# harskish/ganspace

Hardware: NVIDIA H100
Metric: latent samples/sec into PCA (StyleGAN2-ffhq W, N=1e6) (higher is better)
Workload: dtype f32

## Files before the change

### ganspace_b200/csrc/subspace.cu

```cuda
#include "ipca_internal.cuh"
#include <math.h>
#include <stdlib.h>
#include <string.h>

namespace gsb {

constexpr int SC_CL = 16;
constexpr int SC_WARPS = 8;
constexpr int SC_THREADS = SC_WARPS * 32;
constexpr int SC_KT = 32;
constexpr int SC_LDA = SC_KT + 4;
constexpr int SC_STAGES = 3;
constexpr int SC_NB = 5;
constexpr int SC_MAXG = 2;

struct SubspaceParams {
    double *hdr, *mean, *unnorm, *H, *Qbuf;
    const double *mean_b, *gram_b;
    double *Gt, *Part, *Red, *Slots;
    double *Prof;
    int d, c;
    double n_seen, n_b, tol;
    double dbl;
    int maxit;
    int *status;
};

__device__ __forceinline__ void dmma884(double &c0, double &c1, double a, double b) {
    asm("mma.sync.aligned.m8n8k4.row.col.f64.f64.f64.f64 {%0,%1}, {%2}, {%3}, {%0,%1};" : "+d"(c0), "+d"(c1) : "d"(a), "d"(b));
}
__device__ __forceinline__ void sc_cluster_sync() {
    asm volatile("barrier.cluster.arrive.release.aligned;" ::: "memory");
    asm volatile("barrier.cluster.wait.acquire.aligned;" ::: "memory");
}
__device__ __forceinline__ void cp_async16(double *dst, const double *src) {
    const unsigned sa = (unsigned)__cvta_generic_to_shared(dst);
    asm volatile("cp.async.cg.shared.global [%0], [%1], 16;" ::"r"(sa), "l"(src) : "memory");
}
__device__ __forceinline__ void cta_copy_async(double *dst, const double *src, int ndoubles) {
    for (int ch = threadIdx.x; ch < ndoubles / 2; ch += SC_THREADS) cp_async16(dst + 2 * ch, src + 2 * ch);
}

template <bool AT, bool BT>
__device__ __forceinline__ void mma_group(const double *__restrict__ As, int lda, const double *__restrict__ Bs, int ldb,
                                          int ksteps, int m0, int n0, int nb, double (&acc)[SC_NB][2]) {
    const int lane = threadIdx.x & 31, g = lane >> 2, t = lane & 3;
    const double *ap = AT ? (As + (size_t)t * lda + m0 + g) : (As + (size_t)(m0 + g) * lda + t);
    const double *bp = BT ? (Bs + (size_t)(n0 + g) * ldb + t) : (Bs + (size_t)t * ldb + n0 + g);
    const int astep = AT ? 4 * lda : 4, bstep = BT ? 4 : 4 * ldb, bnext = BT ? 8 * ldb : 8;
#pragma unroll 2
    for (int ks = 0; ks < ksteps; ++ks) {
        const double a = ap[(size_t)ks * astep];
#pragma unroll
        for (int b = 0; b < SC_NB; ++b) {
            if (b < nb) {
                const double bv = bp[(size_t)ks * bstep + (size_t)b * bnext];
                dmma884(acc[b][0], acc[b][1], a, bv);
            }
        }
    }
}

__device__ __forceinline__ double fast_rsqrt(double x) {
    double y;
    asm("rsqrt.approx.ftz.f64 %0, %1;" : "=d"(y) : "d"(x));
    const double h = 0.5 * x;
    double t = fma(-h * y, y, 0.5);
    y = fma(y, t, y);
    t = fma(-h * y, y, 0.5);
    y = fma(y, t, y);
    return y;
}

__device__ __forceinline__ void zero_acc(double (&acc)[SC_NB][2]) {
#pragma unroll
    for (int b = 0; b < SC_NB; ++b) { acc[b][0] = 0.0; acc[b][1] = 0.0; }
}

struct Grouping { int mt, nt, nbsel, ngroups; };
__device__ __forceinline__ Grouping make_grouping(int mt, int nt) {
    Grouping q;
    q.mt = mt; q.nt = nt;
    int nb = (mt * nt + SC_WARPS - 1) / SC_WARPS;
    nb = nb < 1 ? 1 : (nb > SC_NB ? SC_NB : nb);
    q.nbsel = nb;
    q.ngroups = mt * ((nt + nb - 1) / nb);
    return q;
}


template <int RA, int CB>
__device__ __forceinline__ void chol_solve_blocked(const double *__restrict__ Ws, double *__restrict__ Ys, int c, int cp, int RPC,
                                                   double *__restrict__ buf ) {
    const int tid = threadIdx.x, ry = tid >> 4, cx = tid & 15, lane = tid & 31;
    const int nrows = c + RPC, CL = 16 * RA;
    double *P = buf, *XS = buf + (size_t)CL * 9, *Lb = XS + (size_t)CL * 9;
    double A[RA][CB];
#pragma unroll
    for (int a = 0; a < RA; ++a) {
        const int r = ry + 16 * a;
#pragma unroll
        for (int b = 0; b < CB; ++b) {
            const int q = cx + 16 * b;
            double v = 0.0;
            if (r < nrows && q < c) v = (r < c) ? Ws[(size_t)r * cp + q] : Ys[(size_t)(r - c) * cp + q];
            A[a][b] = v;
        }
    }
    const double floor_ = fmax(fabs(Ws[0]) * 1e-26, 1e-300);
    __syncthreads();
    for (int p = 0; p < c / 8; ++p) {
        const int j0 = 8 * p, pb = p >> 1, pc = (p & 1) * 8;
        if (cx >= pc && cx < pc + 8) {
#pragma unroll
            for (int b = 0; b < CB; ++b)
                if (b == pb) {
#pragma unroll
                    for (int a = 0; a < RA; ++a) P[(size_t)(ry + 16 * a) * 9 + (cx - pc)] = A[a][b];
                }
        }
        __syncthreads();
        if (tid < 32) {
            const int l = lane & 7;
            double row[8];
#pragma unroll
            for (int k = 0; k < 8; ++k) row[k] = P[(size_t)(j0 + l) * 9 + k];
#pragma unroll
            for (int j = 0; j < 8; ++j) {
                double piv = __shfl_sync(0xffffffffu, row[j], j);
                if (!(piv > floor_)) piv = floor_;
                const double inv = fast_rsqrt(piv);
                const double lij = row[j] * inv;
#pragma unroll
                for (int k = j + 1; k < 8; ++k) {
                    const double lkj = __shfl_sync(0xffffffffu, lij, k);
                    row[k] = fma(-lij, lkj, row[k]);
                }
                row[j] = lij;
                if (lane == j) Lb[72 + j] = inv;
            }
            if (lane < 8) {
#pragma unroll
                for (int k = 0; k < 8; ++k) Lb[l * 9 + k] = (k <= l) ? row[k] : 0.0;
            }
        }
        __syncthreads();
        for (int r = j0 + 8 + tid; r < nrows; r += SC_THREADS) {
            double x[8];
#pragma unroll
            for (int k = 0; k < 8; ++k) {
                double sacc = P[(size_t)r * 9 + k];
#pragma unroll
                for (int m = 0; m < k; ++m) sacc = fma(-x[m], Lb[k * 9 + m], sacc);
                x[k] = sacc * Lb[72 + k];
            }
#pragma unroll
            for (int k = 0; k < 8; ++k) XS[(size_t)r * 9 + k] = x[k];
            if (r >= c) {
#pragma unroll
                for (int k = 0; k < 8; ++k) Ys[(size_t)(r - c) * cp + j0 + k] = x[k];
            }
        }
        __syncthreads();
        double xr[RA][8];
#pragma unroll
        for (int a = 0; a < RA; ++a) {
            const int r = ry + 16 * a;
            const bool ok = (r >= j0 + 8) && (r < nrows);
#pragma unroll
            for (int k = 0; k < 8; ++k) xr[a][k] = ok ? XS[(size_t)r * 9 + k] : 0.0;
        }
#pragma unroll
        for (int b = 0; b < CB; ++b) {
            const int q = cx + 16 * b;
            if (q >= j0 + 8 && q < c) {
                double xq[8];
#pragma unroll
                for (int k = 0; k < 8; ++k) xq[k] = XS[(size_t)q * 9 + k];
#pragma unroll
                for (int a = 0; a < RA; ++a) {
                    double v = A[a][b];
#pragma unroll
                    for (int k = 0; k < 8; ++k) v = fma(-xr[a][k], xq[k], v);
                    A[a][b] = v;
                }
            }
        }
    }
    __syncthreads();
}

template <int RA, int CB>
__global__ void __launch_bounds__(SC_THREADS, 1)
subspace_step_kernel(const SubspaceParams p) {
    extern __shared__ __align__(16) double sc_smem[];
    const int d = p.d, c = p.c, cp = c + 4, RPC = d / SC_CL, RT = RPC / 8, CT = c / 8, nkt = d / SC_KT;
    const int tid = threadIdx.x, lane = tid & 31, warp = tid >> 5, fg = lane >> 2, ft = lane & 3;
    uint32_t me_u;
    asm volatile("mov.u32 %0, %%cluster_ctarank;" : "=r"(me_u));
    const int me = (int)me_u;

    double *As = sc_smem;
    double *Bs = As + (size_t)SC_STAGES * RPC * SC_LDA;
    double *Ys = Bs + (size_t)SC_STAGES * SC_KT * cp;
    double *Qq = Ys + (size_t)RPC * cp;
    double *Ws = Qq + (size_t)RPC * cp;
    double *mv = Ws + (size_t)c * cp;
    double *red = mv + d;
    double *cholbuf = red + 64;
    long long tprev = clock64();
    double prof[10] = {0, 0, 0, 0, 0, 0, 0, 0, 0, 0};
#define PROF(k) do { const long long tn_ = clock64(); prof[k] += (double)(tn_ - tprev); tprev = tn_; } while (0)

    const double n_seen = p.n_seen, n_b = p.n_b, n_tot = n_seen + n_b;
    int cur = (int)__ldcg(p.hdr + 3);
    double *Qc = p.Qbuf + (size_t)cur * d * cp, *Qn = p.Qbuf + (size_t)(cur ^ 1) * d * cp;
    const size_t tileA = (size_t)RPC * SC_LDA, tileB = (size_t)SC_KT * cp;
    double *Gmine = p.Gt + (size_t)me * nkt * tileA;

    {
        const double f = sqrt((n_seen / n_tot) * n_b);
        for (int i = tid; i < d; i += SC_THREADS) mv[i] = f * (__ldcg(p.mean + i) - __ldcg(p.mean_b + i));
        const double *src = Qc + (size_t)me * RPC * cp;
        for (int i = tid; i < RPC * cp; i += SC_THREADS) Qq[i] = __ldcg(src + i);
        for (int i = tid; i < c * c; i += SC_THREADS) Ws[(i / c) * cp + i % c] = __ldcg(p.H + i);
    }
    __syncthreads();
    {
        const Grouping gr = make_grouping(RT, CT);
        for (int g = warp; g < gr.ngroups; g += SC_WARPS) {
            const int rt = g % gr.mt, ct0 = (g / gr.mt) * gr.nbsel;
            const int nb = (gr.nt - ct0 < gr.nbsel) ? gr.nt - ct0 : gr.nbsel;
            double acc[SC_NB][2];
            zero_acc(acc);
            mma_group<false, false>(Qq, cp, Ws, cp, c / 4, rt * 8, ct0 * 8, nb, acc);
#pragma unroll
            for (int b = 0; b < SC_NB; ++b)
                if (b < nb) {
                    double *o = Ys + (size_t)(rt * 8 + fg) * cp + (ct0 + b) * 8 + 2 * ft;
                    o[0] = acc[b][0]; o[1] = acc[b][1];
                }
        }
    }
    __syncthreads();
    PROF(0);
    {
        const Grouping gr = make_grouping(RT, SC_KT / 8);
        auto copy_c = [&](int stage, int kt_) {
            double *dstc = As + (size_t)stage * tileA;
            for (int ch = tid; ch < RPC * (SC_KT / 2); ch += SC_THREADS) {
                const int r = ch / (SC_KT / 2), o2 = ch % (SC_KT / 2);
                cp_async16(dstc + (size_t)r * SC_LDA + 2 * o2, p.gram_b + (size_t)(me * RPC + r) * d + kt_ * SC_KT + 2 * o2);
            }
        };
        for (int s = 0; s < SC_STAGES - 1; ++s) {
            if (s < nkt) { cta_copy_async(Bs + (size_t)s * tileB, Qc + (size_t)s * tileB, (int)tileB); copy_c(s, s); }
            asm volatile("cp.async.commit_group;" ::: "memory");
        }
        for (int kt = 0; kt < nkt; ++kt) {
            asm volatile("cp.async.wait_group %0;" ::"n"(SC_STAGES - 2) : "memory");
            __syncthreads();
            {
                const int nx = kt + SC_STAGES - 1;
                if (nx < nkt) {
                    cta_copy_async(Bs + (size_t)(nx % SC_STAGES) * tileB, Qc + (size_t)nx * tileB, (int)tileB);
                    copy_c(nx % SC_STAGES, nx);
                }
                asm volatile("cp.async.commit_group;" ::: "memory");
            }
            const double *Bt = Bs + (size_t)(kt % SC_STAGES) * tileB, *Cst = As + (size_t)(kt % SC_STAGES) * tileA;
            for (int g = warp; g < gr.ngroups; g += SC_WARPS) {
                const int rt = g % gr.mt, ct0 = (g / gr.mt) * gr.nbsel;
                const int nb = (gr.nt - ct0 < gr.nbsel) ? gr.nt - ct0 : gr.nbsel;
                double acc[SC_NB][2];
                zero_acc(acc);
                mma_group<false, true>(Ys, cp, Bt, cp, c / 4, rt * 8, ct0 * 8, nb, acc);
                const int lrow = rt * 8 + fg, grow = me * RPC + lrow;
                const double mr = mv[grow];
#pragma unroll
                for (int b = 0; b < SC_NB; ++b)
                    if (b < nb) {
                        const int lcol = (ct0 + b) * 8 + 2 * ft, gcol = kt * SC_KT + lcol;
                        const double2 cb = *reinterpret_cast<const double2 *>(Cst + (size_t)lrow * SC_LDA + lcol);
                        double2 o;
                        o.x = acc[b][0] + cb.x + mr * mv[gcol];
                        o.y = acc[b][1] + cb.y + mr * mv[gcol + 1];
                        *reinterpret_cast<double2 *>(Gmine + (size_t)kt * tileA + (size_t)lrow * SC_LDA + lcol) = o;
                    }
            }
        }
        asm volatile("cp.async.wait_group 0;" ::: "memory");
    }
    __syncthreads();
    PROF(1);

    const Grouping gy = make_grouping(RT, CT);
    const Grouping gh = make_grouping(CT, CT);
    const int E = 2 * c * c, slice = (E + SC_CL - 1) / SC_CL;
    double rel = 0.0;
    int it = 0;
    bool conv = false;
    auto gemm_into_ys = [&](const double *Bsrc) {
        {
        double acc[SC_MAXG][SC_NB][2];
#pragma unroll
        for (int q = 0; q < SC_MAXG; ++q) zero_acc(acc[q]);
        for (int s = 0; s < SC_STAGES - 1; ++s) {
            if (s < nkt) {
                cta_copy_async(As + (size_t)s * tileA, Gmine + (size_t)s * tileA, (int)tileA);
                cta_copy_async(Bs + (size_t)s * tileB, Bsrc + (size_t)s * tileB, (int)tileB);
            }
            asm volatile("cp.async.commit_group;" ::: "memory");
        }
        for (int kt = 0; kt < nkt; ++kt) {
            asm volatile("cp.async.wait_group %0;" ::"n"(SC_STAGES - 2) : "memory");
            __syncthreads();
            {
                const int nx = kt + SC_STAGES - 1;
                if (nx < nkt) {
                    cta_copy_async(As + (size_t)(nx % SC_STAGES) * tileA, Gmine + (size_t)nx * tileA, (int)tileA);
                    cta_copy_async(Bs + (size_t)(nx % SC_STAGES) * tileB, Bsrc + (size_t)nx * tileB, (int)tileB);
                }
                asm volatile("cp.async.commit_group;" ::: "memory");
            }
            const double *At = As + (size_t)(kt % SC_STAGES) * tileA, *Bt = Bs + (size_t)(kt % SC_STAGES) * tileB;
#pragma unroll
            for (int q = 0; q < SC_MAXG; ++q) {
                const int g = warp + q * SC_WARPS;
                if (g < gy.ngroups) {
                    const int rt = g % gy.mt, ct0 = (g / gy.mt) * gy.nbsel;
                    const int nb = (gy.nt - ct0 < gy.nbsel) ? gy.nt - ct0 : gy.nbsel;
                    mma_group<false, false>(At, SC_LDA, Bt, cp, SC_KT / 4, rt * 8, ct0 * 8, nb, acc[q]);
                }
            }
        }
        asm volatile("cp.async.wait_group 0;" ::: "memory");
#pragma unroll
        for (int q = 0; q < SC_MAXG; ++q) {
            const int g = warp + q * SC_WARPS;
            if (g < gy.ngroups) {
                const int rt = g % gy.mt, ct0 = (g / gy.mt) * gy.nbsel;
                const int nb = (gy.nt - ct0 < gy.nbsel) ? gy.nt - ct0 : gy.nbsel;
#pragma unroll
                for (int b = 0; b < SC_NB; ++b)
                    if (b < nb) {
                        double *o = Ys + (size_t)(rt * 8 + fg) * cp + (ct0 + b) * 8 + 2 * ft;
                        o[0] = acc[q][b][0]; o[1] = acc[q][b][1];
                    }
            }
        }
    }
    };
    auto partial_reduce = [&]() {
    {
        double *Ph = p.Part + (size_t)me * E, *Pw = Ph + (size_t)c * c;
        for (int g = warp; g < gh.ngroups; g += SC_WARPS) {
            const int mt = g % gh.mt, ct0 = (g / gh.mt) * gh.nbsel;
            const int nb = (gh.nt - ct0 < gh.nbsel) ? gh.nt - ct0 : gh.nbsel;
            double ah[SC_NB][2], aw[SC_NB][2];
            zero_acc(ah); zero_acc(aw);
            mma_group<true, false>(Qq, cp, Ys, cp, RPC / 4, mt * 8, ct0 * 8, nb, ah);
            mma_group<true, false>(Ys, cp, Ys, cp, RPC / 4, mt * 8, ct0 * 8, nb, aw);
#pragma unroll
            for (int b = 0; b < SC_NB; ++b)
                if (b < nb) {
                    const size_t o = (size_t)(mt * 8 + fg) * c + (ct0 + b) * 8 + 2 * ft;
                    *reinterpret_cast<double2 *>(Ph + o) = make_double2(ah[b][0], ah[b][1]);
                    *reinterpret_cast<double2 *>(Pw + o) = make_double2(aw[b][0], aw[b][1]);
                }
        }
    }
    __syncthreads();
    sc_cluster_sync();
    for (int q0 = 0; q0 < slice; q0 += 4 * SC_THREADS) {
        double v[4][SC_CL];
#pragma unroll
        for (int u = 0; u < 4; ++u) {
            const int el = me * slice + q0 + u * SC_THREADS + tid;
            const bool ok = (q0 + u * SC_THREADS + tid < slice) && el < E;
#pragma unroll
            for (int r = 0; r < SC_CL; ++r) v[u][r] = ok ? __ldcg(p.Part + (size_t)r * E + el) : 0.0;
        }
#pragma unroll
        for (int u = 0; u < 4; ++u) {
            const int el = me * slice + q0 + u * SC_THREADS + tid;
            if ((q0 + u * SC_THREADS + tid < slice) && el < E) {
                double s = 0.0;
#pragma unroll
                for (int r = 0; r < SC_CL; ++r) s += v[u][r];
                p.Red[el] = s;
            }
        }
    }
    __syncthreads();
    sc_cluster_sync();
    };
    for (;;) {
        gemm_into_ys(Qc);
        __syncthreads();
        PROF(2);
        partial_reduce();
        for (int i = tid; i < c * c; i += SC_THREADS) Ws[(i / c) * cp + i % c] = __ldcg(p.Red + i);
        __syncthreads();
        PROF(4);
        double rs = 0.0;
        for (int g = warp; g < gy.ngroups; g += SC_WARPS) {
            const int rt = g % gy.mt, ct0 = (g / gy.mt) * gy.nbsel;
            const int nb = (gy.nt - ct0 < gy.nbsel) ? gy.nt - ct0 : gy.nbsel;
            double acc[SC_NB][2];
            zero_acc(acc);
            mma_group<false, false>(Qq, cp, Ws, cp, c / 4, rt * 8, ct0 * 8, nb, acc);
#pragma unroll
            for (int b = 0; b < SC_NB; ++b)
                if (b < nb) {
                    const double *y = Ys + (size_t)(rt * 8 + fg) * cp + (ct0 + b) * 8 + 2 * ft;
                    const double r0 = y[0] - acc[b][0], r1 = y[1] - acc[b][1];
                    rs = fma(r0, r0, rs);
                    rs = fma(r1, r1, rs);
                }
        }
        rs = block_sum(rs, red);
        if (tid == 0) p.Slots[me] = rs;
        __syncthreads();
        sc_cluster_sync();
        {
            double sl[SC_CL];
#pragma unroll
            for (int r = 0; r < SC_CL; ++r) sl[r] = __ldcg(p.Slots + r);
            double hmin = 1e300;
            for (int i = lane; i < c; i += 32) hmin = fmin(hmin, Ws[(size_t)i * cp + i]);
            for (int o = 16; o > 0; o >>= 1) hmin = fmin(hmin, __shfl_xor_sync(0xffffffffu, hmin, o));
            double tot = 0.0;
#pragma unroll
            for (int r = 0; r < SC_CL; ++r) tot += sl[r];
            rel = (hmin > 0.0) ? sqrt(tot) / hmin : 1e300;
            conv = rel <= p.tol;
        }
        PROF(5);
        if (conv || it >= p.maxit) break;
        ++it;
        if (rel > p.dbl * p.tol && it < p.maxit) {
            double *dst = Qn + (size_t)me * RPC * cp;
            for (int i = tid; i < RPC * cp; i += SC_THREADS) dst[i] = ((i % cp) < c) ? Ys[i] : 0.0;
            __syncthreads();
            sc_cluster_sync();
            gemm_into_ys(Qn);
            __syncthreads();
            partial_reduce();
            ++it;
            PROF(2);
        }
        for (int i = tid; i < c * c; i += SC_THREADS) Ws[(i / c) * cp + i % c] = __ldcg(p.Red + (size_t)c * c + i);
        __syncthreads();
        chol_solve_blocked<RA, CB>(Ws, Ys, c, cp, RPC, cholbuf);
        PROF(6);
        {
            double *dst = Qn + (size_t)me * RPC * cp;
            for (int i = tid; i < RPC * cp; i += SC_THREADS) {
                const double v = ((i % cp) < c) ? Ys[i] : 0.0;
                Qq[i] = v;
                dst[i] = v;
            }
        }
        __syncthreads();
        sc_cluster_sync();
        { double *t_ = Qc; Qc = Qn; Qn = t_; }
        cur ^= 1;
        PROF(7);
    }
    if (me == 0) {
        for (int i = tid; i < c * c; i += SC_THREADS) {
            const int a = i / c, b = i % c;
            p.H[i] = 0.5 * (Ws[(size_t)a * cp + b] + Ws[(size_t)b * cp + a]);
        }
    }
    for (int l = tid; l < RPC; l += SC_THREADS) {
        const int i = me * RPC + l;
        const double mb = __ldcg(p.mean_b + i), vb = __ldcg(p.gram_b + (size_t)i * d + i), mo = __ldcg(p.mean + i);
        const double r = n_seen / n_b;
        const double tq = (mo * n_seen) / r - mb * n_b;
        p.unnorm[i] = __ldcg(p.unnorm + i) + vb + r / n_tot * tq * tq;
        p.mean[i] = (mo * n_seen + mb * n_b) / n_tot;
    }
    __syncthreads();
    if (me == 0 && tid == 0) {
        p.hdr[0] = n_tot;
        p.hdr[1] += 1.0;
        p.hdr[2] = 1.0;
        p.hdr[3] = (double)cur;
        p.hdr[4] = (double)it;
        p.hdr[5] = rel;
        p.hdr[6] = fmax(p.hdr[6], rel);
        p.hdr[7] += (double)it;
        if (!conv) atomicOr(p.status, 2);
        PROF(8);
        for (int q = 0; q < 9; ++q) p.Prof[q] += prof[q];
        p.Prof[9] += (double)it;
        p.Prof[10] += 1.0;
    }
    __syncthreads();
    sc_cluster_sync();
}
#undef PROF

__global__ void to_subspace_kernel(double *hdr, const double *__restrict__ S, const double *__restrict__ V, double *__restrict__ H,
                                   double *__restrict__ Qbuf, int d, int c) {
    const int cp = c + 4;
    const size_t idx = blockIdx.x * (size_t)blockDim.x + threadIdx.x;
    if (idx < (size_t)d * cp) {
        const int i = (int)(idx / cp), t = (int)(idx % cp);
        Qbuf[idx] = (t < c) ? V[(size_t)t * d + i] : 0.0;
    }
    if (idx < (size_t)c * c) {
        const int a = (int)(idx / c), b = (int)(idx % c);
        H[idx] = (a == b) ? S[a] * S[a] : 0.0;
    }
    if (idx == 0) { hdr[2] = 1.0; hdr[3] = 0.0; hdr[4] = 0.0; hdr[5] = 0.0; hdr[6] = 0.0; hdr[7] = 0.0; }
}

__global__ void embed_h_kernel(const double *__restrict__ hdr, const double *__restrict__ H, int c, int n, double *__restrict__ A) {
    if (hdr[2] == 0.0) {
        for (int i = threadIdx.x; i < n * n; i += blockDim.x) A[i] = (i / n == i % n) ? -(double)(i / n + 1) : 0.0;
        return;
    }
    __shared__ double red[64];
    double m = 0.0;
    for (int i = threadIdx.x; i < c * c; i += blockDim.x) m = fmax(m, fabs(H[i]));
    for (int o = 16; o > 0; o >>= 1) m = fmax(m, __shfl_xor_sync(0xffffffffu, m, o));
    if ((threadIdx.x & 31) == 0) red[threadIdx.x >> 5] = m;
    __syncthreads();
    m = 0.0;
    for (int q = 0; q < (int)(blockDim.x >> 5); ++q) m = fmax(m, red[q]);
    const double padv = -(m * c + 1.0);
    for (int i = threadIdx.x; i < n * n; i += blockDim.x) {
        const int a = i / n, b = i % n;
        A[i] = (a < c && b < c) ? H[(size_t)a * c + b] : ((a == b) ? padv : 0.0);
    }
}

constexpr int ROT_T = 8;
__global__ void __launch_bounds__(128)
rotate_kernel(const double *__restrict__ hdr, const double *__restrict__ Z, int n, const double *__restrict__ lam,
              const double *__restrict__ Qbuf, int d, int c, double *__restrict__ V, double *__restrict__ S) {
    if (hdr[2] == 0.0) return;
    __shared__ double zs[ROT_T][132];
    const int cp = c + 4, t0 = blockIdx.y * ROT_T;
    const double *Q = Qbuf + (size_t)((int)hdr[3]) * d * cp;
    for (int k = threadIdx.x; k < ROT_T * c; k += blockDim.x) {
        const int t = k / c, sidx = k % c;
        zs[t][sidx] = (t0 + t < c) ? Z[(size_t)(t0 + t) * n + sidx] : 0.0;
    }
    __syncthreads();
    if (blockIdx.x == 0 && threadIdx.x < ROT_T && t0 + threadIdx.x < c) S[t0 + threadIdx.x] = sqrt(fmax(lam[t0 + threadIdx.x], 0.0));
    const int i = blockIdx.x * blockDim.x + threadIdx.x;
    if (i >= d) return;
    const double *qrow = Q + (size_t)i * cp;
    double acc0[ROT_T], acc1[ROT_T];
#pragma unroll
    for (int t = 0; t < ROT_T; ++t) acc0[t] = acc1[t] = 0.0;
    int sidx = 0;
    for (; sidx + 1 < c; sidx += 2) {
        const double q0 = qrow[sidx], q1 = qrow[sidx + 1];
#pragma unroll
        for (int t = 0; t < ROT_T; ++t) { acc0[t] = fma(zs[t][sidx], q0, acc0[t]); acc1[t] = fma(zs[t][sidx + 1], q1, acc1[t]); }
    }
    if (sidx < c) {
        const double q0 = qrow[sidx];
#pragma unroll
        for (int t = 0; t < ROT_T; ++t) acc0[t] = fma(zs[t][sidx], q0, acc0[t]);
    }
#pragma unroll
    for (int t = 0; t < ROT_T; ++t)
        if (t0 + t < c) V[(size_t)(t0 + t) * d + i] = acc0[t] + acc1[t];
}

bool subspace_applicable(int d, int c) {
    if (chain_forced_direct()) return false;
    static int mode = -1;
    if (mode == -1) {
        const char *env = getenv("GANSPACE_B200_CHAIN");
        mode = (env && strcmp(env, "direct") == 0) ? 0 : 1;
    }
    return mode == 1 && d % 128 == 0 && d >= 128 && d <= 512 && c % 8 == 0 && c >= 8 && c <= 128 && 2 * c <= d + d / 4 &&
           subspace_smem_bytes(d, c) <= 227 * 1024;
}

size_t subspace_smem_bytes(int d, int c) {
    const int cp = c + 4, RPC = d / SC_CL;
    return ((size_t)SC_STAGES * RPC * SC_LDA + (size_t)SC_STAGES * SC_KT * cp + 2 * (size_t)RPC * cp + (size_t)c * cp + d + 64 +
            2 * 16 * 10 * 9 + 80) * sizeof(double);
}

SubspaceWs carve_subspace(void *base, int d, int c) {
    SubspaceWs w;
    char *p = reinterpret_cast<char *>(base);
    size_t off = 0;
    auto take = [&](size_t bytes) { char *q = p + off; off += align_up(bytes, 256); return q; };
    const int RPC = d / SC_CL, nkt = d / SC_KT;
    w.Gt = (double *)take((size_t)SC_CL * nkt * RPC * SC_LDA * 8);
    w.Part = (double *)take((size_t)SC_CL * 2 * c * c * 8);
    w.Red = (double *)take((size_t)2 * c * c * 8);
    w.Slots = (double *)take(SC_CL * 8);
    w.bytes = off;
    return w;
}

static double double_step_factor() {
    static double f = -1.0;
    if (f < 0.0) {
        const char *e = getenv("GANSPACE_B200_SUBSPACE_DBL");
        f = e ? atof(e) : 10.0;
        if (!(f > 0.0)) f = 1e300;
    }
    return f;
}

int subspace_step(double *hdr, double *mean, double *unnorm, double *H, double *Qbuf, const double *mean_b, const double *gram_b,
                  const SubspaceWs &w, int d, int c, double n_seen, double n_b, cudaStream_t st) {
    static double tol = -1.0;
    static int maxit = 0;
    if (tol < 0.0) {
        const char *e1 = getenv("GANSPACE_B200_SUBSPACE_TOL"), *e2 = getenv("GANSPACE_B200_SUBSPACE_MAXIT");
        tol = e1 ? atof(e1) : 1e-4;
        if (!(tol > 0.0)) tol = 1e-4;
        maxit = e2 ? atoi(e2) : 60;
        if (maxit < 1) maxit = 60;
    }
    const size_t smem = subspace_smem_bytes(d, c);
    const bool small = (c <= 80 && c + d / SC_CL <= 112);
    auto kern = small ? subspace_step_kernel<7, 5> : subspace_step_kernel<10, 8>;
    static bool cluster_set[2] = {false, false};
    if (!cluster_set[small]) {
        GSB_CHECK_CUDA(cudaFuncSetAttribute(kern, cudaFuncAttributeNonPortableClusterSizeAllowed, 1));
        cluster_set[small] = true;
    }
    if (int r = raise_dyn_smem(kern, smem)) return r;
    SubspaceParams p;
    p.hdr = hdr; p.mean = mean; p.unnorm = unnorm; p.H = H; p.Qbuf = Qbuf;
    p.mean_b = mean_b; p.gram_b = gram_b;
    p.Gt = w.Gt; p.Part = w.Part; p.Red = w.Red; p.Slots = w.Slots; p.Prof = hdr + 8;
    p.d = d; p.c = c; p.n_seen = n_seen; p.n_b = n_b; p.tol = tol; p.maxit = maxit; p.dbl = double_step_factor();
    p.status = eig_status_device_ptr();
    GSB_CHECK_ARG(p.status, "subspace_step: no device status word");
    cudaLaunchConfig_t cfg{};
    cfg.gridDim = dim3(SC_CL); cfg.blockDim = dim3(SC_THREADS); cfg.dynamicSmemBytes = smem; cfg.stream = st;
    cudaLaunchAttribute at[1];
    at[0].id = cudaLaunchAttributeClusterDimension;
    at[0].val.clusterDim.x = SC_CL; at[0].val.clusterDim.y = 1; at[0].val.clusterDim.z = 1;
    cfg.attrs = at; cfg.numAttrs = 1;
    GSB_CHECK_CUDA(cudaLaunchKernelEx(&cfg, kern, p));
    return GSB_OK;
}

int to_subspace_form(double *hdr, const double *S, const double *V, double *H, double *Qbuf, int d, int c, cudaStream_t st) {
    const size_t tot = (size_t)d * (c + 4);
    to_subspace_kernel<<<(unsigned)((tot + 255) / 256), 256, 0, st>>>(hdr, S, V, H, Qbuf, d, c);
    GSB_CHECK_LAUNCH();
    return GSB_OK;
}

int materialise_components(double *hdr, double *S, double *V, const double *H, const double *Qbuf, void *eig_ws, int d, int c,
                           cudaStream_t st) {
    const int n = (c + 31) / 32 * 32;
    Workspace w = carve(eig_ws, n, c);
    embed_h_kernel<<<1, 256, 0, st>>>(hdr, H, c, n, w.A);
    GSB_CHECK_LAUNCH();
    if (int r = eig_top(w, n, c, w.lam, w.evecs, st)) return r;
    GSB_CHECK_ARG(c <= 128, "materialise_components: c <= 128");
    rotate_kernel<<<dim3((unsigned)((d + 127) / 128), (unsigned)((c + ROT_T - 1) / ROT_T)), 128, 0, st>>>(hdr, w.evecs, n, w.lam, Qbuf, d,
                                                                                                    c, V, S);
    GSB_CHECK_LAUNCH();
    return sign_rows(V, c, d, st);
}

}
```

Measured before the change: 18.87 million.

## Fuse first Y=G*Q product into Gram assembly pipeline, skip first gemm_into_ys

While assembling each k-tile of the updated Gram block, the finished tile is written back into the staged shared-memory buffer and immediately multiplied by the resident Q tile to accumulate Y. The first iteration's separate gemm_into_ys pass, which reloads G and Q from global memory, is then skipped. This saves one full streaming pass over the Gram rows per subspace solve. In exchange it adds an extra __syncthreads per k-tile and more accumulator registers during assembly.

```diff
diff --git a/ganspace_b200/csrc/subspace.cu b/ganspace_b200/csrc/subspace.cu
--- a/ganspace_b200/csrc/subspace.cu
+++ b/ganspace_b200/csrc/subspace.cu
@@ -244,7 +244,38 @@
     }
     __syncthreads();
     PROF(0);
+    const Grouping gy = make_grouping(RT, CT);
+    auto y_stage = [&](const double *At, const double *Bt, double (&acc)[SC_MAXG][SC_NB][2]) {
+#pragma unroll
+        for (int q = 0; q < SC_MAXG; ++q) {
+            const int g = warp + q * SC_WARPS;
+            if (g < gy.ngroups) {
+                const int rt = g % gy.mt, ct0 = (g / gy.mt) * gy.nbsel;
+                const int nb = (gy.nt - ct0 < gy.nbsel) ? gy.nt - ct0 : gy.nbsel;
+                mma_group<false, false>(At, SC_LDA, Bt, cp, SC_KT / 4, rt * 8, ct0 * 8, nb, acc[q]);
+            }
+        }
+    };
+    auto store_y = [&](const double (&acc)[SC_MAXG][SC_NB][2]) {
+#pragma unroll
+        for (int q = 0; q < SC_MAXG; ++q) {
+            const int g = warp + q * SC_WARPS;
+            if (g < gy.ngroups) {
+                const int rt = g % gy.mt, ct0 = (g / gy.mt) * gy.nbsel;
+                const int nb = (gy.nt - ct0 < gy.nbsel) ? gy.nt - ct0 : gy.nbsel;
+#pragma unroll
+                for (int b = 0; b < SC_NB; ++b)
+                    if (b < nb) {
+                        double *o = Ys + (size_t)(rt * 8 + fg) * cp + (ct0 + b) * 8 + 2 * ft;
+                        o[0] = acc[q][b][0]; o[1] = acc[q][b][1];
+                    }
+            }
+        }
+    };
     {
+        double yacc[SC_MAXG][SC_NB][2];
+#pragma unroll
+        for (int q = 0; q < SC_MAXG; ++q) zero_acc(yacc[q]);
         const Grouping gr = make_grouping(RT, SC_KT / 8);
         auto copy_c = [&](int stage, int kt_) {
             double *dstc = As + (size_t)stage * tileA;
@@ -268,7 +299,8 @@
                 }
                 asm volatile("cp.async.commit_group;" ::: "memory");
             }
-            const double *Bt = Bs + (size_t)(kt % SC_STAGES) * tileB, *Cst = As + (size_t)(kt % SC_STAGES) * tileA;
+            const double *Bt = Bs + (size_t)(kt % SC_STAGES) * tileB;
+            double *Cst = As + (size_t)(kt % SC_STAGES) * tileA;
             for (int g = warp; g < gr.ngroups; g += SC_WARPS) {
                 const int rt = g % gr.mt, ct0 = (g / gr.mt) * gr.nbsel;
                 const int nb = (gr.nt - ct0 < gr.nbsel) ? gr.nt - ct0 : gr.nbsel;
@@ -286,15 +318,19 @@
                         o.x = acc[b][0] + cb.x + mr * mv[gcol];
                         o.y = acc[b][1] + cb.y + mr * mv[gcol + 1];
                         *reinterpret_cast<double2 *>(Gmine + (size_t)kt * tileA + (size_t)lrow * SC_LDA + lcol) = o;
+                        *reinterpret_cast<double2 *>(Cst + (size_t)lrow * SC_LDA + lcol) = o;
                     }
             }
+            __syncthreads();
+            y_stage(Cst, Bt, yacc);
         }
         asm volatile("cp.async.wait_group 0;" ::: "memory");
+        __syncthreads();
+        store_y(yacc);
     }
     __syncthreads();
     PROF(1);
 
-    const Grouping gy = make_grouping(RT, CT);
     const Grouping gh = make_grouping(CT, CT);
     const int E = 2 * c * c, slice = (E + SC_CL - 1) / SC_CL;
     double rel = 0.0;
@@ -395,8 +431,8 @@
     __syncthreads();
     sc_cluster_sync();
     };
-    for (;;) {
-        gemm_into_ys(Qc);
+    for (bool first = true;; first = false) {
+        if (!first) gemm_into_ys(Qc);
         __syncthreads();
         PROF(2);
         partial_reduce();
```

Result: no change. 19.13 million, median of 6 (+1.4%).
